# AwesomePeiweiPan/Droid-SLAM_Reserch

Hardware: AMD Instinct MI355X
Metric: BA update iters/sec (2000-edge equivalents; 256 keyframes, 48x64) (higher is better)
Workload: dtype f32; 1 GPU; 256-keyframe / 2000-edge global BA, 48x64, t0=1, lm=1e-5 ep=1e-2 (BASELINE configs[2]); edges_total=2000, solve=fp64 dense Cholesky on device, chol_failed=False

## Files before the change

droid-slam_reserch_amd/csrc/api.hip:

```cpp
#include <hip/hip_runtime.h>
#include <stdio.h>
#include <string.h>

#include <algorithm>
#include <map>
#include <mutex>

#include "../../include/droid_backends_hip.h"
#include "ba_internal.hpp"
#include "graph.hpp"

namespace droid {
int launch_corr_index_forward(const void* volume, const float* coords, void* corr, int B, int H1,
                              int W1, int H2, int W2, int r, int dtype, hipStream_t s);
int launch_corr_pyramid_forward(const void* const* volumes, const float* coords, void* corr, int B, int H1, int W1,
                                int r, int levels, int dtype, hipStream_t s);
int launch_corr_pyramid_forward_slots(const void* const* volumes, const int64_t* slots, long long cap, const float* coords,
                                      void* corr, int B, int H1, int W1, int r, int levels, int dtype, hipStream_t s);
int launch_corr_index_backward(const float* coords, const void* corr_grad, void* volume_grad, int B,
                               int H1, int W1, int H2, int W2, int r, int dtype, hipStream_t s);
int launch_altcorr_pyramid_forward(const void* const* levels_dev, const int64_t* ii, const int64_t* jj,
                                   const float* coords, float* corr, int E, int frames, int H, int W, int C,
                                   int r, int nlevels, int dtype, hipStream_t s);
int launch_altcorr_forward(const void* f1, const void* f2, const float* coords, void* corr, int B,
// ... 327 lines not shown
    b = (nc + 1 == max_chunks || b + size >= nb) ? nb : b + size;
    bcol[++nc] = b;
    if (++ones >= 2) size++;
  }
  return nc;
}

int droid_ba_overlap_plan(int t0, int t1, int max_chunks, int* nchunks_out, size_t* packed_offsets) {
  if (t1 <= t0 || max_chunks < 1 || max_chunks > 32 || !nchunks_out || !packed_offsets)
    return fail(DROID_E_ARG, "ba_overlap_plan: bad %s", "argument");
  const int n = 6 * (t1 - t0);
  int brow[33];
  const int nc = overlap_bounds(n, max_chunks, brow);
  const int nb = (n + CHOL_NB - 1) / CHOL_NB;
  for (int c = 0; c <= nc; c++) packed_offsets[c] = brow[c] >= nb ? pk_total(n) : pk_colbase(n, brow[c]);
  *nchunks_out = nc;
  return DROID_OK;
}

int droid_ba_unpack_chunk(int E, int nbuf, int H, int W, int M, int t0, int t1, int chunk, int max_chunks, float lm,
                          float ep, int epoch, void* workspace, size_t workspace_bytes, void* stream) {
  BaView v;
  int rc = ba_view(v, workspace, workspace_bytes, E, nbuf, H, W, t0, t1, M, 0);
  if (rc) return rc;
  int brow[33];
  if (max_chunks < 1 || max_chunks > 32) return fail(DROID_E_ARG, "ba_unpack_chunk: bad %s", "max_chunks");
  const int nc = overlap_bounds(v.n, max_chunks, brow);
  if (chunk < 0 || chunk >= nc || epoch <= 0) return fail(DROID_E_ARG, "ba_unpack_chunk: bad %s", "chunk / epoch");
  launch_unpack_cols(v, brow[chunk], brow[chunk + 1], (double)lm, (double)ep, epoch, (hipStream_t)stream);
  return check_hip("ba_unpack_chunk");
}

static int solve_update_check(const float* poses, const float* disps, const float* intrinsics, const float* weights,
                              const int64_t* ii, const int64_t* jj, int E, int motion_only) {
  if (!poses || !disps) return fail(DROID_E_ARG, "ba: null %s", "state pointer");
  if (!motion_only && (!intrinsics || (E > 0 && (!weights || !ii || !jj))))
    return fail(DROID_E_ARG, "ba: null %s", "intrinsics/weights/edges");
  return DROID_OK;
}

int droid_ba_solve_update_overlap(float* poses, float* disps, const float* intrinsics, const float* weights,
                                  const int64_t* ii, const int64_t* jj, int E, int nbuf, int H, int W, int M,
                                  int t0, int t1, int epoch, int motion_only, float* dx_out, float* dz_out,
                                  void* workspace, size_t workspace_bytes, void* stream) {
  BaView v;
  int rc = ba_view(v, workspace, workspace_bytes, E, nbuf, H, W, t0, t1, M, motion_only);
  if (!rc) rc = solve_update_check(poses, disps, intrinsics, weights, ii, jj, E, motion_only);
  if (rc) return rc;
  if (E <= 0 || epoch <= 0) return fail(DROID_E_ARG, "ba_solve_update_overlap: needs %s", "edges (the build presets the solver scratch) and epoch > 0");
  hipStream_t s = (hipStream_t)stream;
  const CholSystem c(v);
  if (!launch_chol_factor_overlap(c, v.ov_ready, epoch, s))
    return fail(DROID_E_ARG, "ba_solve_update_overlap: %s", "the single-launch solver is not available for this system (unpack and call droid_ba_solve_update)");
  launch_chol_backsolve(c, true, s);
  launch_update(v, poses, disps, intrinsics, weights, ii, jj, v.xsol, dx_out, dz_out, motion_only != 0, s,
                mirror_of(workspace));
  return check_hip("ba_solve_update_overlap");
}

int droid_ba_solve_update(float* poses, float* disps, const float* intrinsics, const float* weights,
                          const int64_t* ii, const int64_t* jj, int E, int nbuf, int H, int W, int M,
                          int t0, int t1, float lm, float ep, int motion_only, float* dx_out,
                          float* dz_out, void* workspace, size_t workspace_bytes, void* stream) {
  BaView v;
  int rc = ba_view(v, workspace, workspace_bytes, E, nbuf, H, W, t0, t1, M, motion_only);
  if (!rc) rc = solve_update_check(poses, disps, intrinsics, weights, ii, jj, E, motion_only);
  if (rc) return rc;
  hipStream_t s = (hipStream_t)stream;
  launch_chol_solve(CholSystem(v), (double)lm, (double)ep, s, E > 0);
  launch_update(v, poses, disps, intrinsics, weights, ii, jj, v.xsol, dx_out, dz_out, motion_only != 0, s,
                mirror_of(workspace));
  return check_hip("ba_solve_update");
}

int droid_ba(float* poses, float* disps, const float* intrinsics, const float* disps_sens,
             const float* targets, const float* weights, const float* eta, const int64_t* ii,
             const int64_t* jj, int E, int nbuf, int H, int W, int M, int t0, int t1,
             int iterations, float lm, float ep, int motion_only, float* dx_out, float* dz_out,
             void* workspace, size_t workspace_bytes, void* stream) {
  int rc = droid_ba_prepare(ii, jj, E, nbuf, H, W, M, t0, t1, 0, nbuf, motion_only, workspace,
                            workspace_bytes, stream);
  if (rc) return rc;
  for (int it = 0; it < iterations; it++) {
    rc = droid_ba_build(poses, disps, intrinsics, disps_sens, targets, weights, eta, ii, jj, E,
                        nbuf, H, W, M, t0, t1, motion_only, workspace, workspace_bytes, stream);
    if (rc) return rc;
    rc = droid_ba_solve_update(poses, disps, intrinsics, weights, ii, jj, E, nbuf, H, W, M, t0, t1, lm, ep, motion_only,
                               dx_out, dz_out, workspace, workspace_bytes, stream);
    if (rc) return rc;
  }
  return DROID_OK;
}

int droid_ba_profile_iteration(float* poses, float* disps, const float* intrinsics,
                               const float* disps_sens, const float* targets, const float* weights,
                               const float* eta, const int64_t* ii, const int64_t* jj, int E,
                               int nbuf, int H, int W, int M, int t0, int t1, float lm, float ep,
                               int motion_only, void* workspace, size_t workspace_bytes,
                               void* stream, float* stage_ms) {
  BaView v;
  int rc = ba_view(v, workspace, workspace_bytes, E, nbuf, H, W, t0, t1, M, motion_only);
  if (rc) return rc;
  hints_of(v, workspace, false);
  if (!stage_ms) return fail(DROID_E_ARG, "ba_profile: null %s", "stage_ms");
  hipStream_t s = (hipStream_t)stream;
  hipEvent_t ev[7];
  for (auto& e : ev) (void)hipEventCreate(&e);
// ... 183 lines not shown
```

droid-slam_reserch_amd/csrc/ba_internal.hpp:

```cpp
#pragma once
#include <hip/hip_runtime.h>
#include <stddef.h>
#include <stdint.h>

namespace droid {

constexpr int LIN_THREADS = 256;
constexpr int LIN_PPT = 2;
constexpr int LIN_CP = LIN_THREADS * LIN_PPT;
constexpr int CHOL_NB = 64;
__host__ __device__ inline int chol_ld(int n) { return (n + 1 + 15) & ~15; }
__host__ __device__ inline size_t chol_flag_words(int n) { return 2 * ((size_t)(n + 1 + CHOL_NB - 1) / CHOL_NB) + 8; }
__host__ __device__ inline int chol_tile_index(int nrb, int bi, int bj) { return bj * nrb - bj * (bj - 1) / 2 + (bi - bj); }
__host__ __device__ inline size_t chol_tiles(int n) {
  const int nb = (n + CHOL_NB - 1) / CHOL_NB, nrb = (n + 1 + CHOL_NB - 1) / CHOL_NB;
  return (size_t)chol_tile_index(nrb, nb, nb);
}
__host__ __device__ inline size_t chol_mbuf_offset(int n) { return ((size_t)(n + CHOL_NB - 1) / CHOL_NB) * CHOL_NB * CHOL_NB; }
__host__ __device__ inline size_t chol_lfin_offset(int n) { return 2 * chol_mbuf_offset(n); }
__host__ __device__ inline size_t chol_ldiag_doubles(int n) { return chol_lfin_offset(n) + chol_tiles(n) * CHOL_NB * CHOL_NB; }

__host__ __device__ inline size_t pk_colbase(int n, int J) {
  return (size_t)CHOL_NB * ((size_t)J * (size_t)(n + 1) - (size_t)CHOL_NB * (size_t)J * (size_t)(J - 1) / 2);
}
__host__ __device__ inline int pk_width(int n, int J) { return (n - CHOL_NB * J) < CHOL_NB ? (n - CHOL_NB * J) : CHOL_NB; }
__host__ __device__ inline size_t pk_total(int n) {
  if (n <= 0) return 0;
  const int nb = (n + CHOL_NB - 1) / CHOL_NB;
  return pk_colbase(n, nb - 1) + (size_t)(n + 1 - CHOL_NB * (nb - 1)) * (size_t)pk_width(n, nb - 1);
}
__host__ __device__ inline size_t pk_index(int n, int gi, int gj) {
  const int J = gj / CHOL_NB;
  return pk_colbase(n, J) + (size_t)(gi - CHOL_NB * J) * (size_t)pk_width(n, J) + (size_t)(gj - CHOL_NB * J);
}
__host__ __device__ inline unsigned pk_index32(int n, int gi, int gj) {
  const int J = gj >> 6, c0 = J << 6;
  const int w = (n - c0) < CHOL_NB ? (n - c0) : CHOL_NB;
  return (unsigned)(CHOL_NB * (J * (n + 1) - (CHOL_NB / 2) * J * (J - 1)) + (gi - c0) * w + (gj - c0));
}

enum { HDR_STATUS = 0, HDR_M = 1, HDR_CHOL_FAIL = 2, HDR_NENT = 3, HDR_NWORK = 4,
       HDR_NC1 = 5, HDR_NC2 = 6,
       HDR_WORDS = 16 };
enum { STATUS_BAD_INDEX = 1, STATUS_ETA_ROWS = 2, STATUS_CHOL_FAIL = 4, STATUS_CHOL_STALL = 8 };

struct BaView {
  int E, nbuf, H, W, HW;
  int t0, t1, P, M;
  int n, ld;
  int nch;
  int own0, own1;
  int motion_only;
  int* hdr;
  int* slot_of;
  int* kx;
  int* seg_ptr;
  int* seg_edge;
  int* cursor;
  int* ent_ptr;
  int* ent_row;
  int* ent_pose;
  int* wk_ptr;
  int* order;
  int* xtmp;
  int* cls_list;
  int* gt_ptr;
  double* Gpart;
  int s2_split;
  float* Hpart;
  float* Q;
  float* w;
  float* Erows;
  float* Ebuf;
// ... 74 lines not shown
    v.zsplit = z < 1 ? 1 : (z > 8 ? 8 : z);
  }
  v.zpart = nullptr;
  if (v.zsplit > 1) v.zpart = static_cast<float*>(take(sizeof(float) * ((size_t)v.zsplit * M * 8 * v.HW + 64)));
  v.s2_split = 1;
  v.Gpart = nullptr;
  if (M > 0) {
    const int ptiles = (v.HW + 63) / 64;
    int ns = S2_WGS / M;
    v.s2_split = ns < 1 ? 1 : (ns > ptiles ? ptiles : ns);
    size_t tiles = (size_t)E * 7 / 4 + (size_t)M + 1;
    if (tiles > (size_t)28 * M) tiles = (size_t)28 * M;
    v.Gpart = static_cast<double*>(take(sizeof(double) * (tiles * v.s2_split * 256 + 64)));
  }
  v.sys = static_cast<double*>(take(sizeof(double) * ((size_t)(v.n + 1) * v.ld + 8)));
  v.psys = static_cast<double*>(take(sizeof(double) * (pk_total(v.n) + 8)));
  v.packed = 0;
  v.xsol = static_cast<double*>(take(sizeof(double) * ((size_t)v.ld + 1)));
  v.bs_flags = static_cast<int*>(take(sizeof(int) * chol_flag_words(v.n)));
  v.ldiag = static_cast<double*>(take(sizeof(double) * chol_ldiag_doubles(v.n)));
  v.dx = static_cast<float*>(take(sizeof(float) * ((size_t)v.n + 8)));
  v.ov_ready = static_cast<int*>(take(sizeof(int) * ((size_t)(v.n + 1 + CHOL_NB - 1) / CHOL_NB + 8)));
  return off;
}

__host__ __device__ inline int solver_preset_words(const BaView& v) {
  return (int)((reinterpret_cast<const char*>(v.bs_flags) - reinterpret_cast<const char*>(v.xsol)) / 4 +
               (long)chol_flag_words(v.n));
}
__host__ __device__ inline int solver_preset_tiles(const BaView& v) { return v.n > 0 ? (int)chol_tiles(v.n) : 0; }

struct CholSystem {
  double* S; int n, ld; double* x; int* flags; double* ldiag; int* fail;
  explicit CholSystem(const BaView& v)
      : S(v.sys), n(v.n), ld(v.ld), x(v.xsol), flags(v.bs_flags), ldiag(v.ldiag), fail(v.hdr + HDR_CHOL_FAIL) {}
  CholSystem(double* scratch, int n, double* x, int* fail);
  static size_t scratch_doubles(int n);
};

void launch_prep(const BaView& v, const int64_t* ii, const int64_t* jj, hipStream_t s);
void launch_unpack_system(const BaView& v, hipStream_t s);
void launch_build(const BaView& v, const float* poses, const float* disps, const float* intr,
                  const float* sens, const float* targets, const float* weights, const float* eta,
                  const int64_t* ii, const int64_t* jj, bool motion_only, hipStream_t s);
void launch_build_stage(const BaView& v, const float* poses, const float* disps, const float* intr,
                        const float* sens, const float* targets, const float* weights,
                        const float* eta, const int64_t* ii, const int64_t* jj, bool motion_only,
                        int stage, hipStream_t s);
void launch_update(const BaView& v, float* poses, float* disps, const float* intr, const float* weights,
                   const int64_t* ii, const int64_t* jj, const double* x, float* dx_out, float* dz_out,
                   bool motion_only, hipStream_t s, int* status_mirror = nullptr);
void launch_chol_preset(const CholSystem& c, hipStream_t s);
bool launch_chol_factor(const CholSystem& c, double lm, double ep, hipStream_t s);
void launch_chol_backsolve(const CholSystem& c, bool factor_single, hipStream_t s);
void launch_chol_solve(const CholSystem& c, double lm, double ep, hipStream_t s, bool preset_done);

void launch_unpack_cols(const BaView& v, int J0, int J1, double lm, double ep, int epoch, hipStream_t s);
bool launch_chol_factor_overlap(const CholSystem& c, const int* ready, int epoch, hipStream_t s);

}
```

droid-slam_reserch_amd/csrc/chol.hip:

```cpp
#include <hip/hip_runtime.h>
#include <mutex>

#include <cstdint>
#include <cstdlib>

#include "ba_internal.hpp"

namespace droid {

constexpr int NB = CHOL_NB;

#ifdef CHOL_STAMPS
__device__ unsigned long long g_chol_stamps[64 * 16];
__shared__ unsigned long long g_chol_lstamps[16];
#define STAMP(slot)                                                                         \
  do {                                                                                      \
    if (!PERSIST && threadIdx.x == 0 && panel && (blockIdx.x < 2)) {                                     \
      g_chol_stamps[((k + 1) & 31) * 32 + blockIdx.x * 16 + (slot)] = __builtin_amdgcn_s_memtime(); \
    }                                                                                       \
    if (PERSIST && threadIdx.x == 0 && panel && (bi - kp < 2)) {                              \
       \
      g_chol_lstamps[slot] = wall_clock64();                                                  \
      if ((slot) == 2) { g_chol_lstamps[14] = 0; g_chol_lstamps[15] = 0; g_chol_lstamps[9] = 0; }                    \
      if ((slot) == 8)                                                                        \
// ... 572 lines not shown
      if (wave < nd) {
        const int q = p + 1 + wave;
        wave_gemm_nt16<true>(&B2[(16 * q) * LDP + 16 * p], &B2[(16 * q) * LDP + 16 * p], &Wl[WLB * p], WLP);
      } else if (solve_rows && wave < nd + 4) {
        const int g = wave - nd;
        wave_gemm_nt16<true>(&BT[(16 * g) * LDP + 16 * p], &BT[(16 * g) * LDP + 16 * p], &Wl[WLB * p], WLP);
      }
    }
    if (p == 0) STAMP(10);
    __syncthreads();
    if (p == 0) STAMP(5);
    if (PERSIST && solve_rows && wave == 4)
      chol_strip_out(S, ld, Ldiag + chol_lfin_offset(n) + (size_t)chol_tile_index((nrows + NB - 1) / NB, bi, kp) * NB * NB, BT,
                     r0, c0, wk, nrows, p, (p == 3) ? &done[bi] : nullptr, 4 * kp + 3);
    if (p == 3) break;
    const int q = p + 1;
    if (wave == 0) {
      wave_gemm_nt16<false>(&B2[(16 * q) * LDP + 16 * q], &B2[(16 * q) * LDP + 16 * p],
                            &B2[(16 * q) * LDP + 16 * p], LDP);
      wave_potrf16(&B2[(16 * q) * LDP + 16 * q], &Wl[WLB * q], Idn, fail, diag);
      if (p == 0) STAMP(6);
    } else {
      int cnt = 0;
#pragma unroll 1
      for (int r = q; r < 4; r++)
#pragma unroll 1
        for (int s2 = q; s2 <= r; s2++) {
          if (r == q && s2 == q) continue;
          {
            const int slot = cnt % 2;
            const int owner = 1 + slot + ((1 + slot >= q) ? 1 : 0);
            if (owner == wave)
              wave_gemm_nt16<false>(&B2[(16 * r) * LDP + 16 * s2], &B2[(16 * r) * LDP + 16 * p],
                                    &B2[(16 * s2) * LDP + 16 * p], LDP);
          }
          cnt++;
        }
      const bool mine = (wave >= 5) ? (ndef > 0) : (ndef > 0 && wave == q);
      if (mine) {
        f64x4 acc = dacc[0];
        if (!PERSIST && k >= 0) strip_update_tile(acc, B0, B1, dg, q);
#pragma unroll
        for (int pp = 0; pp < 3; pp++)
          if (pp <= p) block_update16(acc, &BT[(16 * dg) * LDP + 16 * pp], &B2[(16 * q) * LDP + 16 * pp]);
        store_solve(acc, dg, q);
        dacc[0] = dacc[1];
        dacc[1] = dacc[2];
      }
    }
    __syncthreads();
    if (p == 0) STAMP(7);
  }
  STAMP(8);
  if (PERSIST && bi == kp + 1 && kp + 1 < (n + NB - 1) / NB) {
    __syncthreads();
    if (wave < 4) {
      const int g = wave;
#pragma unroll
      for (int q = 3; q >= 0; q--) {
        lds_f64* Cq = &BT[(16 * g) * LDP + 16 * q];
        f64x4 acc;
#pragma unroll
        for (int i = 0; i < 4; i++) acc[i] = Cq[(fg + 4 * i) * LDP + fr];
#pragma unroll
        for (int s2 = q + 1; s2 < 4; s2++)
#pragma unroll
          for (int kk = 0; kk < 16; kk += 4)
            acc = __builtin_amdgcn_mfma_f64_16x16x4f64(-BT[(16 * g + fr) * LDP + 16 * s2 + kk + fg],
                                                       B2[(16 * s2 + kk + fg) * LDP + 16 * q + fr], acc, 0, 0, 0);
#pragma unroll
        for (int i = 0; i < 4; i++) Cq[(fg + 4 * i) * LDP + fr] = acc[i];
        f64x4 m = {0.0, 0.0, 0.0, 0.0};
#pragma unroll
        for (int kk = 0; kk < 16; kk += 4)
          m = __builtin_amdgcn_mfma_f64_16x16x4f64(Cq[fr * LDP + kk + fg], Wl[WLB * q + (kk + fg) * WLP + fr], m, 0, 0, 0);
#pragma unroll
        for (int i = 0; i < 4; i++) Cq[(fg + 4 * i) * LDP + fr] = m[i];
      }
      gbl_f64* Mj = Ldiag + chol_mbuf_offset(n) + (size_t)kp * NB * NB;
#pragma unroll
      for (int it = 0; it < 8; it++) {
        const int u = it * 64 + lane;
        const int i = 16 * g + (u >> 5), j2 = (u & 31) * 2;
        f64x2 v = *(const lds_f64x2*)&BT[i * LDP + j2];
        if (r0 + i >= n) v = (f64x2){0.0, 0.0};
        *(gbl_f64x2*)&Mj[i * NB + j2] = v;
      }
    }
  }
  if (PERSIST && diag) {
#pragma unroll
    for (int e = t; e < 1024; e += 512) {
      const int pb = e >> 8, j = (e >> 4) & 15, kk = e & 15;
      const int br = pb == 3 ? 1 : 0, bc = pb == 3 ? 2 : pb + 1;
      B2[(16 * br + j) * LDP + 16 * bc + kk] = Wl[WLB * pb + WLP * j + kk];
    }
    __syncthreads();
  }
  if (grp == 0) {
    if (diag) {
      if (PERSIST) store_tile64(Ldiag + (size_t)kp * NB * NB, B2, NB, 0, 0, 0, NB, NB, false);
      else store_tile64(S, B2, ld, c0, c0, c0, c0 + wk, wk, true);
    }
  } else if (solve_rows && !PERSIST) {
    store_tile64(S, BT, ld, r0, c0, max(r0, c0 + wk), min(r0 + NB, nrows), wk, false);
  }
  if (!PERSIST) STAMP(9);
}

__global__ __launch_bounds__(512) void chol_step_kernel(double* __restrict__ S, int n, int ld, int k,
                                                        int* __restrict__ fail, double lm, double ep) {
  chol_tile<false>((gbl_f64*)S, n, ld, k, k + 1 + (int)blockIdx.x, k + 1 + (int)blockIdx.y, fail, lm, ep, nullptr,
                   nullptr, nullptr);
}


template <bool OV>
__device__ __attribute__((noinline)) void chol_tile_persist(double* __restrict__ S, int n, int ld, int k, int bi,
                                                            int bj, int* __restrict__ fail, double lm, double ep,
                                                            double* __restrict__ Ldiag, int* __restrict__ done,
                                                            int* __restrict__ abortf, bool coh_first, int k_last) {
  chol_tile<true, OV>((gbl_f64*)S, n, ld, k, bi, bj, fail, lm, ep, (gbl_f64*)Ldiag, done, abortf, coh_first, k_last);
}

#ifdef OV_DEBUG
__device__ unsigned long long g_ov_dbg[64];
extern "C" int droid_debug_overlap_stamps(unsigned long long* out) {
  return (int)hipMemcpyFromSymbol(out, HIP_SYMBOL(g_ov_dbg), sizeof(unsigned long long) * 64);
}
#endif
template <bool OV>
__global__ __launch_bounds__(512) void chol_factor_persistent_kernel(double* __restrict__ S, int n, int ld,
                                                                     int* __restrict__ fail, double lm, double ep,
                                                                     int* __restrict__ flags,
                                                                     double* __restrict__ Ldiag,
                                                                     const int* __restrict__ ready_arg, int epoch) {
  const int* const ready = OV ? ready_arg : nullptr;
  __shared__ int s_abort;
  const int nb = (n + NB - 1) / NB;
  const int nrb = (n + 1 + NB - 1) / NB;
  int* done = flags;
  int* dver = flags + nrb;
  int* abortf = flags + 2 * nrb;
  const int G = (int)gridDim.x, wg = (int)blockIdx.x, t = (int)threadIdx.x;
  int total = 0;
  for (int j = 0; j < nb; j++) total += nrb - j;

  {
    int cs = 0;
    for (int j = 0; j < nb; j++) {
      if (j >= 1 && (cs % G) == wg) {
        const int i = j * NB + t;
        if (ready == nullptr && t < NB && i < n) {
          const double d = S[(size_t)i * ld + i];
          gstore<true>((gbl_f64*)&S[(size_t)i * ld + i], d + (ep + lm * d));
        }
        asm volatile("s_waitcnt vmcnt(0)" ::: "memory");
        __syncthreads();
        if (t == 0) cfp_store(&dver[j], 0);
      }
      cs += nrb - j;
    }
  }

#ifdef OV_DEBUG
  if (blockIdx.x == 0 && threadIdx.x == 0) g_ov_dbg[63] = wall_clock64();
#endif
  if (OV && ready != nullptr) {
    constexpr int MAXT = 12;
    __shared__ int s_ti[MAXT], s_tj[MAXT], s_nx[MAXT], s_nt, s_pick, s_klast;
    if (t == 0) {
      int nt = 0, cj = 0, cs = 0;
      for (int idx = wg; idx < total && nt < MAXT; idx += G) {
        while (idx >= cs + (nrb - cj)) {
          cs += nrb - cj;
          cj++;
        }
        s_ti[nt] = cj + (idx - cs);
        s_tj[nt] = cj;
        s_nx[nt] = (cj == 0) ? -1 : 0;
        nt++;
      }
      s_nt = nt;
    }
    __syncthreads();
    while (true) {
      if (t < 64) {
        int pick = -1, spins = 0, klast = -2;
        bool ok = true;
        const int nt = s_nt;
        while (true) {
          bool any_left = false;
          for (int i = 0; i < nt; i++) {
            const int bi = s_ti[i], bj = s_tj[i], k = s_nx[i];
            if (k > bj - 1) continue;
            any_left = true;
            const int kp = k + 1;
            const bool panel = (bj == kp);
            const bool first = (k == ((bj == 0) ? -1 : 0));
// ... 75 lines not shown
      }
      const int bj = __builtin_amdgcn_readfirstlane(cj), bi = __builtin_amdgcn_readfirstlane(cj + (idx - cs));
      if (k < 0 && bj != 0) break;
      const bool panel = (bj == kp);
      PSTAMP(11);
      const bool first_touch = (ready != nullptr) && (k <= 0);
      if (t < 64) {
        bool ok = true;
        if (k >= 0 || first_touch) {
          const int* p = nullptr;
          int need = 4 * k + 3;
          const bool flagged = k >= 0 && !panel && bj != kp + 1;
          if (t == 0 && flagged) p = &done[bi];
          else if (t == 1 && flagged && bj != bi) p = &done[bj];
          else if (t == 2 && k >= 0 && panel && bi != bj) { p = &dver[bj]; need = k; }
          else if (t == 3 && first_touch) { p = &ready[bj]; need = epoch; }
          bool sat = (p == nullptr);
          int spins = 0;
          const int limit = (ready != nullptr) ? (CFP_SPIN_LIMIT << 4) : CFP_SPIN_LIMIT;
          while (true) {
            if (!sat) sat = cfp_load(p) >= need;
            if (__all(sat)) break;
            spins++;
            if (spins > limit || ((spins & 255) == 0 && __any(cfp_load(abortf) == 1))) {
              ok = false;
              break;
            }
            if (ready != nullptr) __builtin_amdgcn_s_sleep(4);
            else __builtin_amdgcn_s_sleep(1);
          }
        } else if (__any(cfp_load(abortf) == 1)) {
          ok = false;
        }
        if (t == 0) {
          s_abort = ok ? 0 : 1;
          if (!ok) {
            cfp_store(abortf, 1);
            atomicMax(fail, 2);
          }
        }
      }
      PSTAMP(12);
      __syncthreads();
      if (s_abort) return;
      chol_tile_persist<false>(S, n, ld, k, bi, bj, fail, lm, ep, Ldiag, done, abortf, false, k);
      if (!panel && bi == bj) {
        asm volatile("s_waitcnt vmcnt(0)" ::: "memory");
        __syncthreads();
        if (t == 0) cfp_store(&dver[bj], k + 1);
      }
      PSTAMP(13);
    }
    colstart += nrb - kp;
  }
}

__global__ __launch_bounds__(256) void chol_backsolve_kernel(double* __restrict__ S, int n, int ld,
                                                             int k, double* __restrict__ x) {
  __shared__ double L[NB * LDP];
  __shared__ double xk[NB];
  const int t = threadIdx.x;
  const int c0 = k * NB;
  const int wk = min(NB, n - c0);
  load_tile64(DROID_LDS(L), (const gbl_f64*)S, ld, c0, c0, c0, c0 + wk, c0 + wk, true, 1.0);
  __syncthreads();
  if (t < 64) {
    double z = (t < wk) ? S[(size_t)n * ld + c0 + t] : 0.0;
    const double rinv = 1.0 / L[t * LDP + t];
#pragma unroll
    for (int i = NB - 1; i >= 0; i--) {
      const double xi = readlane_f64(z * rinv, i);
      z = (t == i) ? xi : ((t < i) ? fma(-L[i * LDP + t], xi, z) : z);
    }
    xk[t] = z;
  }
  __syncthreads();
  if (blockIdx.x == 0) {
    if (t < wk) x[c0 + t] = xk[t];
    return;
  }
  const int c = (blockIdx.x - 1) * 256 + t;
  if (c < c0) {
    double s4[4] = {0.0, 0.0, 0.0, 0.0};
    const double* col = S + (size_t)c0 * ld + c;
#pragma unroll
    for (int r = 0; r < NB; r += 16) {
      double v[16];
#pragma unroll
      for (int u = 0; u < 16; u++) v[u] = (r + u < wk) ? col[(size_t)(r + u) * ld] : 0.0;
#pragma unroll
      for (int u = 0; u < 16; u++) s4[u & 3] = fma(v[u], xk[r + u], s4[u & 3]);
    }
    S[(size_t)n * ld + c] -= (s4[0] + s4[1]) + (s4[2] + s4[3]);
  }
}

constexpr int BSP_MAX_BLOCKS = 200;
#ifdef CHOL_STAMPS
__device__ unsigned long long g_bs_stamps[64 * 8];
#define BSTAMP(slot) do { if (threadIdx.x == 0 && blockIdx.x < 64) g_bs_stamps[blockIdx.x * 8 + (slot)] = wall_clock64(); } while (0)
#else
#define BSTAMP(slot) do { } while (0)
#endif
constexpr long long BSP_SENTINEL = -1LL;

__device__ __forceinline__ void load_tile64_w123(lds_f64* __restrict__ dst, const gbl_f64* __restrict__ S,
                                                 int ld, int r0, int c0, int row_end, int col_end) {
// ... 156 lines not shown
        u0 = fma(Lcol[16 * B + ii], xx[0], u0);                                                        \
        u1 = fma(Lcol[16 * B + ii + 1], xx[1], u1);                                                    \
      }                                                                                                \
      z -= u0 + u1;                                                                                    \
    }
    DROID_BS_BLOCK(3)
    DROID_BS_BLOCK(2)
    DROID_BS_BLOCK(1)
    DROID_BS_BLOCK(0)
#undef DROID_BS_BLOCK
#undef DROID_BS_WTERM
#undef DROID_BS_STEP
    BSTAMP(2);
    if (FAST && j < nb - 1) xsol -= poll_matvec(j + 1, Mc);
    if (__double_as_longlong(xsol) == BSP_SENTINEL) xsol = __longlong_as_double(0x7ff8000000000000LL);
    BSTAMP(4);
    if (t < wj) __hip_atomic_store(&x[c0 + t], xsol, __ATOMIC_RELAXED, __HIP_MEMORY_SCOPE_AGENT);
    BSTAMP(5);
  }
}


struct CholSwitches {
  bool multi_launch;
  bool cooperative;
  bool force_bs_refusal;
  int grid;
  int overlap_reserve;
};
static const CholSwitches& chol_switches() {
  static const CholSwitches sw = {
      getenv("DROID_CHOL_MULTI_LAUNCH") != nullptr,
      getenv("DROID_CHOL_COOPERATIVE") != nullptr && atoi(getenv("DROID_CHOL_COOPERATIVE")) != 0,
      getenv("DROID_CHOL_FORCE_BS_REFUSAL") != nullptr,
      getenv("DROID_CHOL_GRID") ? atoi(getenv("DROID_CHOL_GRID")) : 0,
      getenv("DROID_OVERLAP_RESERVE_CUS") ? atoi(getenv("DROID_OVERLAP_RESERVE_CUS")) : 32};
  return sw;
}

static int chol_resident_workgroups() {
  static int cached = -1;
  if (cached < 0) {
    int dev = 0, occ = 0;
    hipDeviceProp_t prop;
    if (hipGetDevice(&dev) != hipSuccess || hipGetDeviceProperties(&prop, dev) != hipSuccess ||
        hipOccupancyMaxActiveBlocksPerMultiprocessor(&occ, chol_factor_persistent_kernel<false>, 512, 0) != hipSuccess)
      cached = 0;
    else
      cached = occ * prop.multiProcessorCount;
  }
  return cached;
}

static bool chol_single_launch(const CholSystem& c) {
  const int nb = (c.n + NB - 1) / NB;
  return !chol_switches().multi_launch && nb >= 2 && (c.ld % 16) == 0 && (reinterpret_cast<uintptr_t>(c.S) % 128) == 0 &&
         chol_resident_workgroups() >= 8 && chol_tiles(c.n) <= (size_t)10 * chol_resident_workgroups();
}

static int chol_factor_grid(int n, int cap) { return chol_tiles(n) < (size_t)cap ? (int)chol_tiles(n) : cap; }

struct PersistState {
  hipStream_t last = nullptr;
  hipEvent_t ev = nullptr;
  bool any = false;
};
static PersistState g_persist[64];
static std::mutex g_persist_mu;

static std::unique_lock<std::mutex> persist_enter(hipStream_t s) {
  std::unique_lock<std::mutex> lock(g_persist_mu);
  int dev = 0;
  if (hipGetDevice(&dev) != hipSuccess || dev < 0 || dev >= 64) return lock;
  PersistState& st = g_persist[dev];
  if (st.any && st.last != s) {
    if (!st.ev && hipEventCreateWithFlags(&st.ev, hipEventDisableTiming) != hipSuccess) st.ev = nullptr;
    if (st.ev && hipEventRecord(st.ev, st.last) == hipSuccess) (void)hipStreamWaitEvent(s, st.ev, 0);
    (void)hipGetLastError();
  }
  st.last = s;
  st.any = true;
  return lock;
}

__global__ __launch_bounds__(256) void chol_ldiag_to_sys_kernel(double* __restrict__ S, int n, int ld,
                                                                const double* __restrict__ Ldiag) {
  const int j = blockIdx.x, c0 = j * NB, wk = min(NB, n - c0);
  for (int idx = threadIdx.x; idx < NB * NB; idx += blockDim.x) {
    const int i = idx / NB, c = idx % NB;
    if (i < wk && c <= i) S[(size_t)(c0 + i) * ld + c0 + c] = Ldiag[(size_t)j * NB * NB + idx];
  }
}

bool launch_chol_factor_overlap(const CholSystem& c, const int* ready, int epoch, hipStream_t s) {
  const CholSwitches& sw = chol_switches();
  if (c.n <= 0 || !ready || sw.cooperative || !chol_single_launch(c)) return false;
  const int cap = chol_resident_workgroups() - (sw.overlap_reserve > 0 ? sw.overlap_reserve : 0);
  if (cap < 8 || chol_tiles(c.n) > (size_t)10 * cap) return false;
  auto lock = persist_enter(s);
  const double zero = 0.0;
  hipLaunchKernelGGL(chol_factor_persistent_kernel<true>, dim3(chol_factor_grid(c.n, cap)), dim3(512), 0, s, c.S, c.n,
                     c.ld, c.fail, zero, zero, c.flags, c.ldiag, ready, epoch);
  return true;
}

bool launch_chol_factor(const CholSystem& c, double lm, double ep, hipStream_t s) {
  if (c.n <= 0) return false;
  const CholSwitches& sw = chol_switches();
  if (chol_single_launch(c)) {
    int cap = chol_resident_workgroups();
    if (sw.grid >= 8 && sw.grid < cap) cap = sw.grid;
    const dim3 grid(chol_factor_grid(c.n, cap));
    CholSystem a = c;
    const int* no_ready = nullptr;
    int no_epoch = 0;
    void* args[] = {&a.S, &a.n, &a.ld, &a.fail, &lm, &ep, &a.flags, &a.ldiag, &no_ready, &no_epoch};
    const void* fn = (const void*)chol_factor_persistent_kernel<false>;
    auto lock = persist_enter(s);
    if (!sw.cooperative) {
      (void)hipLaunchKernel(fn, grid, dim3(512), args, 0, s);
      return true;
    }
    if (hipLaunchCooperativeKernel(fn, grid, dim3(512), args, 0, s) == hipSuccess) return true;
    (void)hipGetLastError();
  }
  const int nb = (c.n + NB - 1) / NB;
  const int nrb = (c.n + 1 + NB - 1) / NB;
  for (int k = -1; k + 1 < nb; k++)
    hipLaunchKernelGGL(chol_step_kernel, dim3(nrb - k - 1, k < 0 ? 2 : nb - k - 1), dim3(512), 0, s, c.S, c.n,
                       c.ld, k, c.fail, lm, ep);
  return false;
}

void launch_chol_backsolve(const CholSystem& c, bool factor_single, hipStream_t s) {
  const int nb = (c.n + NB - 1) / NB;
  if (nb >= 2 && nb <= BSP_MAX_BLOCKS) {
    const CholSwitches& sw = chol_switches();
    CholSystem a = c;
    const double* ld_arg = factor_single ? c.ldiag : nullptr;
    void* args[] = {&a.S, &a.n, &a.ld, &a.x, &a.fail, &ld_arg};
    const void* fn = factor_single ? (const void*)chol_backsolve_persistent_kernel<true>
                                   : (const void*)chol_backsolve_persistent_kernel<false>;
    auto lock = persist_enter(s);
    if (!sw.cooperative) {
      (void)hipLaunchKernel(fn, dim3(nb), dim3(256), args, 0, s);
      return;
    }
    if (!sw.force_bs_refusal && hipLaunchCooperativeKernel(fn, dim3(nb), dim3(256), args, 0, s) == hipSuccess) return;
    (void)hipGetLastError();
  }
  if (factor_single)
    hipLaunchKernelGGL(chol_ldiag_to_sys_kernel, dim3(nb), dim3(256), 0, s, c.S, c.n, c.ld, c.ldiag);
  for (int k = nb - 1; k >= 0; k--) {
    const int c0 = k * NB;
    hipLaunchKernelGGL(chol_backsolve_kernel, dim3(1 + (c0 + 255) / 256), dim3(256), 0, s, c.S, c.n,
                       c.ld, k, c.x);
  }
}

void launch_chol_preset(const CholSystem& c, hipStream_t s) {
  (void)hipMemsetAsync(c.fail, 0, sizeof(int), s);
  const size_t xbytes = sizeof(double) * (size_t)c.n, fbytes = sizeof(int) * chol_flag_words(c.n);
  const char* xb = reinterpret_cast<const char*>(c.x);
  const char* fb = reinterpret_cast<const char*>(c.flags);
  if (fb >= xb + xbytes && fb - xb <= (ptrdiff_t)(xbytes + 4096)) {
    (void)hipMemsetAsync(c.x, 0xFF, (size_t)(fb - xb) + fbytes, s);
  } else {
    (void)hipMemsetAsync(c.x, 0xFF, xbytes, s);
    (void)hipMemsetAsync(c.flags, 0xFF, fbytes, s);
  }
  (void)hipMemsetAsync(c.ldiag + chol_lfin_offset(c.n), 0xFF, sizeof(double) * chol_tiles(c.n) * NB * NB, s);
}

void launch_chol_solve(const CholSystem& c, double lm, double ep, hipStream_t s, bool preset_done) {
  if (c.n <= 0) return;
  if (!preset_done) launch_chol_preset(c, s);
  const bool single = launch_chol_factor(c, lm, ep, s);
  launch_chol_backsolve(c, single, s);
}

size_t CholSystem::scratch_doubles(int n) {
  if (n <= 0) return 0;
  return (size_t)(n + 1) * chol_ld(n) + chol_ldiag_doubles(n) + (chol_flag_words(n) + 1) / 2 + 16;
}
CholSystem::CholSystem(double* scratch, int n_, double* x_, int* fail_)
    : S(scratch), n(n_), ld(chol_ld(n_)), x(x_), fail(fail_) {
  ldiag = S + (size_t)(n + 1) * ld;
  flags = reinterpret_cast<int*>(ldiag + chol_ldiag_doubles(n));
// ... 30 lines not shown
```

Baseline: 1990 iters/s.

## Build inverse Cholesky factor inside persistent factor kernel and replace backsolve with GEMV

Idle workgroups in the persistent Cholesky factor kernel now build the block upper-triangular inverse of L tile by tile (Z tiles), scheduled through new per-column readiness flags. The non-overlapped backsolve becomes a single parallel matrix-vector product with the stored inverse. This replaces the serial block-by-block triangular solve, which has a long dependency chain, at the cost of extra O(n^3) work, more workspace, and more flag polling inside the factor kernel. The overlapped path keeps the old backsolve.

```diff
diff --git a/droid-slam_reserch_amd/csrc/api.hip b/droid-slam_reserch_amd/csrc/api.hip
--- a/droid-slam_reserch_amd/csrc/api.hip
+++ b/droid-slam_reserch_amd/csrc/api.hip
@@ -403,7 +403,7 @@
   const CholSystem c(v);
   if (!launch_chol_factor_overlap(c, v.ov_ready, epoch, s))
     return fail(DROID_E_ARG, "ba_solve_update_overlap: %s", "the single-launch solver is not available for this system (unpack and call droid_ba_solve_update)");
-  launch_chol_backsolve(c, true, s);
+  launch_chol_backsolve(c, true, s, true);
   launch_update(v, poses, disps, intrinsics, weights, ii, jj, v.xsol, dx_out, dz_out, motion_only != 0, s,
                 mirror_of(workspace));
   return check_hip("ba_solve_update_overlap");
diff --git a/droid-slam_reserch_amd/csrc/ba_internal.hpp b/droid-slam_reserch_amd/csrc/ba_internal.hpp
--- a/droid-slam_reserch_amd/csrc/ba_internal.hpp
+++ b/droid-slam_reserch_amd/csrc/ba_internal.hpp
@@ -10,7 +10,7 @@
 constexpr int LIN_CP = LIN_THREADS * LIN_PPT;
 constexpr int CHOL_NB = 64;
 __host__ __device__ inline int chol_ld(int n) { return (n + 1 + 15) & ~15; }
-__host__ __device__ inline size_t chol_flag_words(int n) { return 2 * ((size_t)(n + 1 + CHOL_NB - 1) / CHOL_NB) + 8; }
+__host__ __device__ inline size_t chol_flag_words(int n) { return 4 * ((size_t)(n + 1 + CHOL_NB - 1) / CHOL_NB) + 8; }
 __host__ __device__ inline int chol_tile_index(int nrb, int bi, int bj) { return bj * nrb - bj * (bj - 1) / 2 + (bi - bj); }
 __host__ __device__ inline size_t chol_tiles(int n) {
   const int nb = (n + CHOL_NB - 1) / CHOL_NB, nrb = (n + 1 + CHOL_NB - 1) / CHOL_NB;
@@ -18,7 +18,13 @@
 }
 __host__ __device__ inline size_t chol_mbuf_offset(int n) { return ((size_t)(n + CHOL_NB - 1) / CHOL_NB) * CHOL_NB * CHOL_NB; }
 __host__ __device__ inline size_t chol_lfin_offset(int n) { return 2 * chol_mbuf_offset(n); }
-__host__ __device__ inline size_t chol_ldiag_doubles(int n) { return chol_lfin_offset(n) + chol_tiles(n) * CHOL_NB * CHOL_NB; }
+__host__ __device__ inline size_t chol_zinv_offset(int n) { return chol_lfin_offset(n) + chol_tiles(n) * CHOL_NB * CHOL_NB; }
+__host__ __device__ inline int chol_ztile_index(int nb, int zi, int bj) { return zi * nb - zi * (zi - 1) / 2 + (bj - zi); }
+__host__ __device__ inline size_t chol_ztiles(int n) {
+  const size_t nb = (size_t)(n + CHOL_NB - 1) / CHOL_NB;
+  return nb * (nb + 1) / 2;
+}
+__host__ __device__ inline size_t chol_ldiag_doubles(int n) { return chol_zinv_offset(n) + chol_ztiles(n) * CHOL_NB * CHOL_NB; }
 
 __host__ __device__ inline size_t pk_colbase(int n, int J) {
   return (size_t)CHOL_NB * ((size_t)J * (size_t)(n + 1) - (size_t)CHOL_NB * (size_t)J * (size_t)(J - 1) / 2);
@@ -199,7 +205,7 @@
                    bool motion_only, hipStream_t s, int* status_mirror = nullptr);
 void launch_chol_preset(const CholSystem& c, hipStream_t s);
 bool launch_chol_factor(const CholSystem& c, double lm, double ep, hipStream_t s);
-void launch_chol_backsolve(const CholSystem& c, bool factor_single, hipStream_t s);
+void launch_chol_backsolve(const CholSystem& c, bool factor_single, hipStream_t s, bool overlapped = false);
 void launch_chol_solve(const CholSystem& c, double lm, double ep, hipStream_t s, bool preset_done);
 
 void launch_unpack_cols(const BaView& v, int J0, int J1, double lm, double ep, int epoch, hipStream_t s);
diff --git a/droid-slam_reserch_amd/csrc/chol.hip b/droid-slam_reserch_amd/csrc/chol.hip
--- a/droid-slam_reserch_amd/csrc/chol.hip
+++ b/droid-slam_reserch_amd/csrc/chol.hip
@@ -648,7 +648,7 @@
     if (p == 0) STAMP(7);
   }
   STAMP(8);
-  if (PERSIST && bi == kp + 1 && kp + 1 < (n + NB - 1) / NB) {
+  if (PERSIST && OV && bi == kp + 1 && kp + 1 < (n + NB - 1) / NB) {
     __syncthreads();
     if (wave < 4) {
       const int g = wave;
@@ -695,11 +695,16 @@
   }
   if (grp == 0) {
     if (diag) {
-      if (PERSIST) store_tile64(Ldiag + (size_t)kp * NB * NB, B2, NB, 0, 0, 0, NB, NB, false);
+      if (PERSIST) store_tile64<!OV>(Ldiag + (size_t)kp * NB * NB, B2, NB, 0, 0, 0, NB, NB, false);
       else store_tile64(S, B2, ld, c0, c0, c0, c0 + wk, wk, true);
     }
   } else if (solve_rows && !PERSIST) {
     store_tile64(S, BT, ld, r0, c0, max(r0, c0 + wk), min(r0 + NB, nrows), wk, false);
+  }
+  if (PERSIST && !OV && diag) {
+    asm volatile("s_waitcnt vmcnt(0)" ::: "memory");
+    __syncthreads();
+    if (t == 0) cfp_store(&done[3 * ((nrows + NB - 1) / NB) + 8 + kp], 1);
   }
   if (!PERSIST) STAMP(9);
 }
@@ -718,6 +723,77 @@
                                                             int* __restrict__ abortf, bool coh_first, int k_last) {
   chol_tile<true, OV>((gbl_f64*)S, n, ld, k, bi, bj, fail, lm, ep, (gbl_f64*)Ldiag, done, abortf, coh_first, k_last);
 }
+
+__device__ __attribute__((noinline)) void chol_ztile(const double* __restrict__ S_, int n, int ld,
+                                                     double* __restrict__ Ldiag_, int zi, int bj, int u0, int u1,
+                                                     bool solve, bool fresh) {
+  const gbl_f64* S = (const gbl_f64*)S_;
+  gbl_f64* Ldiag = (gbl_f64*)Ldiag_;
+  lds_f64* const B0 = DROID_LDS(g_cholB0);
+  lds_f64* const B1 = DROID_LDS(g_cholB1);
+  lds_f64* const B2 = DROID_LDS(g_cholB2);
+  lds_f64* const BT = DROID_LDS(g_cholBT);
+  lds_f64* const Wl = DROID_LDS(g_cholWl);
+  const int nb = (n + NB - 1) / NB;
+  gbl_f64* Zbase = Ldiag + chol_zinv_offset(n);
+  gbl_f64* Zt = Zbase + (size_t)chol_ztile_index(nb, zi, bj) * NB * NB;
+  const int t = threadIdx.x, wave = t >> 6, lane = t & 63;
+  const int grp = wave >> 2, w4 = wave & 3;
+  const int fr = lane & 15, fg = lane >> 4;
+  f64x4 acc[4];
+  if (fresh) {
+#pragma unroll
+    for (int nn = 0; nn < 2; nn++)
+#pragma unroll
+      for (int i = 0; i < 4; i++)
+        acc[nn][i] = (zi == bj && 16 * w4 + fg + 4 * i == 16 * (2 * grp + nn) + fr) ? 1.0 : 0.0;
+  } else {
+    frag_load_global<2>(acc, Zt, NB, 0, 0, w4, 2 * grp, NB, NB, false);
+  }
+  for (int kk = u0; kk < u1; kk++) {
+    if (kk > u0) __syncthreads();
+    if (grp == 0) load_tile64<true>(B0, Zbase + (size_t)chol_ztile_index(nb, zi, kk) * NB * NB, NB, 0, 0, 0, NB, NB, false, 0.0);
+    else load_tile64<true>(B1, S, ld, bj * NB, kk * NB, bj * NB, n, kk * NB + NB, false, 0.0);
+    __syncthreads();
+    strip_update<2>(acc, B0, B1, w4, 2 * grp);
+  }
+#pragma unroll
+  for (int nn = 0; nn < 2; nn++)
+#pragma unroll
+    for (int i = 0; i < 4; i++) BT[(16 * w4 + fg + 4 * i) * LDP + 16 * (2 * grp + nn) + fr] = acc[nn][i];
+  if (solve) {
+    if (grp == 1) load_tile64<true>(B2, Ldiag + (size_t)bj * NB * NB, NB, 0, 0, 0, NB, NB, false, 0.0);
+    __syncthreads();
+    for (int e = t; e < 1024; e += 512) {
+      const int pb = e >> 8, j = (e >> 4) & 15, kk = e & 15;
+      const int br = pb == 3 ? 1 : 0, bc = pb == 3 ? 2 : pb + 1;
+      Wl[WLB * pb + WLP * j + kk] = B2[(16 * br + j) * LDP + 16 * bc + kk];
+    }
+    __syncthreads();
+    if (wave < 4) {
+      const int g = wave;
+#pragma unroll
+      for (int p = 0; p < 4; p++) {
+        lds_f64* Cp = &BT[(16 * g) * LDP + 16 * p];
+        if (p > 0) {
+          f64x4 a;
+#pragma unroll
+          for (int i = 0; i < 4; i++) a[i] = Cp[(fg + 4 * i) * LDP + fr];
+#pragma unroll
+          for (int s2 = 0; s2 < 3; s2++)
+            if (s2 < p) block_update16(a, &BT[(16 * g) * LDP + 16 * s2], &B2[(16 * p) * LDP + 16 * s2]);
+#pragma unroll
+          for (int i = 0; i < 4; i++) Cp[(fg + 4 * i) * LDP + fr] = a[i];
+        }
+        wave_gemm_nt16<true>(Cp, Cp, &Wl[WLB * p], WLP);
+      }
+    }
+  }
+  __syncthreads();
+  if (grp == 0) store_tile64<true>(Zt, BT, NB, 0, 0, 0, NB, NB, false);
+  asm volatile("s_waitcnt vmcnt(0)" ::: "memory");
+}
+constexpr int CFP_ZMAX = 64;
 
 #ifdef OV_DEBUG
 __device__ unsigned long long g_ov_dbg[64];
@@ -738,9 +814,97 @@
   int* done = flags;
   int* dver = flags + nrb;
   int* abortf = flags + 2 * nrb;
+  int* zdone = flags + 2 * nrb + 8;
+  int* dfin = zdone + nrb;
   const int G = (int)gridDim.x, wg = (int)blockIdx.x, t = (int)threadIdx.x;
   int total = 0;
   for (int j = 0; j < nb; j++) total += nrb - j;
+
+  __shared__ int s_zi[CFP_ZMAX], s_zj[CFP_ZMAX], s_znx[CFP_ZMAX], s_zpick, s_zu1, s_zsolve;
+  int nz = 0;
+  if (!OV) {
+    const int ztotal = nb * (nb + 1) / 2;
+    nz = (ztotal > wg) ? (ztotal - wg + G - 1) / G : 0;
+    if (nz > CFP_ZMAX) {
+      if (t == 0) {
+        cfp_store(abortf, 1);
+        atomicMax(fail, 2);
+      }
+      nz = 0;
+    }
+    if (t == 0) {
+      int zi = 0, rs = 0;
+      for (int i = 0; i < nz; i++) {
+        const int zidx = wg + i * G;
+        while (zidx >= rs + (nb - zi)) {
+          rs += nb - zi;
+          zi++;
+        }
+        s_zi[i] = zi;
+        s_zj[i] = zi + (zidx - rs);
+        s_znx[i] = zi;
+      }
+    }
+    __syncthreads();
+  }
+  auto z_work = [&](bool drain) -> bool {
+    int budget = nz;
+    while (true) {
+      if (t < 64) {
+        int pick = -1, pu1 = 0, spins = 0;
+        bool psolve = false, ok = true;
+        while (true) {
+          bool any_left = false;
+          for (int i = 0; i < nz; i++) {
+            const int zi = s_zi[i], bj = s_zj[i], u = s_znx[i];
+            if (u > bj) continue;
+            any_left = true;
+            const int zd = cfp_load(&zdone[zi]), dn = cfp_load(&done[bj]), df = cfp_load(&dfin[bj]);
+            int u1 = min(bj, min(zd + 1, ((dn - 3) >> 2) + 1));
+            if (u1 < u) u1 = u;
+            const bool sv = (u1 == bj) && df >= 0;
+            if (u1 > u || sv) {
+              pick = i;
+              pu1 = u1;
+              psolve = sv;
+              break;
+            }
+          }
+          if (!any_left) pick = -2;
+          if (pick != -1 || !drain) break;
+          if (++spins > CFP_SPIN_LIMIT || ((spins & 63) == 0 && cfp_load(abortf) == 1)) {
+            ok = false;
+            break;
+          }
+          __builtin_amdgcn_s_sleep(8);
+        }
+        if (t == 0) {
+          s_zpick = ok ? pick : -3;
+          s_zu1 = pu1;
+          s_zsolve = psolve ? 1 : 0;
+          if (!ok) {
+            cfp_store(abortf, 1);
+            atomicMax(fail, 2);
+          }
+        }
+      }
+      __syncthreads();
+      const int pick = __builtin_amdgcn_readfirstlane(s_zpick);
+      if (pick == -3) return false;
+      if (pick < 0) return true;
+      const int zi = __builtin_amdgcn_readfirstlane(s_zi[pick]), bj = __builtin_amdgcn_readfirstlane(s_zj[pick]);
+      const int u = __builtin_amdgcn_readfirstlane(s_znx[pick]), u1 = __builtin_amdgcn_readfirstlane(s_zu1);
+      const bool sv = __builtin_amdgcn_readfirstlane(s_zsolve) != 0;
+      chol_ztile(S, n, ld, Ldiag, zi, bj, u, u1, sv, u == zi);
+      __syncthreads();
+      if (t == 0) {
+        if (sv) cfp_store(&zdone[zi], bj);
+        s_znx[pick] = sv ? bj + 1 : u1;
+      }
+      __syncthreads();
+      if (!drain && --budget <= 0) return true;
+    }
+  };
 
   {
     int cs = 0;
@@ -922,7 +1086,38 @@
       PSTAMP(13);
     }
     colstart += nrb - kp;
-  }
+    if (!OV && nz > 0 && !z_work(false)) return;
+  }
+  if (!OV && nz > 0) (void)z_work(true);
+}
+
+__global__ __launch_bounds__(256) void chol_apply_inverse_kernel(const double* __restrict__ S, int n, int ld,
+                                                                 double* __restrict__ x, const int* __restrict__ fail,
+                                                                 const double* __restrict__ Z) {
+  const int nb = (int)gridDim.y, zi = (int)blockIdx.y;
+  const int wave = threadIdx.x >> 6, lane = threadIdx.x & 63;
+  const int row = 4 * (int)blockIdx.x + wave;
+  const int gi = zi * NB + row;
+  if (gi >= n) return;
+  if (*fail != 0) {
+    if (lane == 0) x[gi] = 0.0;
+    return;
+  }
+  const int half = lane >> 5, j2 = (lane & 31) * 2;
+  const double* __restrict__ y = S + (size_t)n * ld;
+  double s0 = 0.0, s1 = 0.0;
+#pragma unroll 4
+  for (int bj = zi + half; bj < nb; bj += 2) {
+    const f64x2 z = *(const f64x2*)&Z[(size_t)chol_ztile_index(nb, zi, bj) * NB * NB + row * NB + j2];
+    const int c = bj * NB + j2;
+    const double y0 = (c < n) ? y[c] : 0.0, y1 = (c + 1 < n) ? y[c + 1] : 0.0;
+    s0 = fma(z[0], y0, s0);
+    s1 = fma(z[1], y1, s1);
+  }
+  double sum = s0 + s1;
+#pragma unroll
+  for (int off = 32; off > 0; off >>= 1) sum += __shfl_xor(sum, off);
+  if (lane == 0) x[gi] = sum;
 }
 
 __global__ __launch_bounds__(256) void chol_backsolve_kernel(double* __restrict__ S, int n, int ld,
@@ -1185,10 +1380,11 @@
   return cached;
 }
 
-static bool chol_single_launch(const CholSystem& c) {
+static bool chol_single_launch(const CholSystem& c, bool with_inverse) {
   const int nb = (c.n + NB - 1) / NB;
+  const size_t tiles = chol_tiles(c.n) + (with_inverse ? chol_ztiles(c.n) : 0);
   return !chol_switches().multi_launch && nb >= 2 && (c.ld % 16) == 0 && (reinterpret_cast<uintptr_t>(c.S) % 128) == 0 &&
-         chol_resident_workgroups() >= 8 && chol_tiles(c.n) <= (size_t)10 * chol_resident_workgroups();
+         chol_resident_workgroups() >= 8 && tiles <= (size_t)10 * chol_resident_workgroups();
 }
 
 static int chol_factor_grid(int n, int cap) { return chol_tiles(n) < (size_t)cap ? (int)chol_tiles(n) : cap; }
@@ -1227,7 +1423,7 @@
 
 bool launch_chol_factor_overlap(const CholSystem& c, const int* ready, int epoch, hipStream_t s) {
   const CholSwitches& sw = chol_switches();
-  if (c.n <= 0 || !ready || sw.cooperative || !chol_single_launch(c)) return false;
+  if (c.n <= 0 || !ready || sw.cooperative || !chol_single_launch(c, false)) return false;
   const int cap = chol_resident_workgroups() - (sw.overlap_reserve > 0 ? sw.overlap_reserve : 0);
   if (cap < 8 || chol_tiles(c.n) > (size_t)10 * cap) return false;
   auto lock = persist_enter(s);
@@ -1240,9 +1436,9 @@
 bool launch_chol_factor(const CholSystem& c, double lm, double ep, hipStream_t s) {
   if (c.n <= 0) return false;
   const CholSwitches& sw = chol_switches();
-  if (chol_single_launch(c)) {
+  if (chol_single_launch(c, true)) {
     int cap = chol_resident_workgroups();
-    if (sw.grid >= 8 && sw.grid < cap) cap = sw.grid;
+    if (sw.grid >= 8 && sw.grid < cap && chol_ztiles(c.n) <= (size_t)CFP_ZMAX * sw.grid) cap = sw.grid;
     const dim3 grid(chol_factor_grid(c.n, cap));
     CholSystem a = c;
     const int* no_ready = nullptr;
@@ -1265,8 +1461,13 @@
   return false;
 }
 
-void launch_chol_backsolve(const CholSystem& c, bool factor_single, hipStream_t s) {
+void launch_chol_backsolve(const CholSystem& c, bool factor_single, hipStream_t s, bool overlapped) {
   const int nb = (c.n + NB - 1) / NB;
+  if (factor_single && !overlapped) {
+    hipLaunchKernelGGL(chol_apply_inverse_kernel, dim3(NB / 4, nb), dim3(256), 0, s, c.S, c.n, c.ld, c.x, c.fail,
+                       c.ldiag + chol_zinv_offset(c.n));
+    return;
+  }
   if (nb >= 2 && nb <= BSP_MAX_BLOCKS) {
     const CholSwitches& sw = chol_switches();
     CholSystem a = c;
```

New measurement: 1891 iters/s. -5.0%, worse.
